# KochPJ/AutoPoseEstimation

Measured on AMD Instinct MI355X. Metric: RGB-D frames/sec (seg+DenseFusion+2-refine), 640x480 N=1000, higher is better.
Workload: dtype bf16x3

## Files before the change

autoposeestimation_amd/_lib.py:

```python
import ctypes
import os

import torch

_HERE = os.path.dirname(os.path.abspath(__file__))
LIB_PATH = os.environ.get("APE_HIP_LIB", os.path.join(_HERE, "libape_hip.so"))

_c = ctypes
_P, _I, _F, _L, _D = _c.c_void_p, _c.c_int, _c.c_float, _c.c_int64, _c.c_double

SIGNATURES = {
    "ape_abi_version": [],
    "ape_last_error": [],
    "ape_knn_f32": [_P, _P, _P, _I, _I, _I, _I, _I, _P],
    "ape_conv2d_nhwc_f32": [_P, _P, _P, _P, _P, _P, _P],
    "ape_packed_weights_bf16_elems": [_I, _I],
    "ape_pack_weights_bf16": [_P, _P, _I, _I, _P],
    "ape_conv2d_nhwc_bf16": [_P, _P, _P, _P, _P, _P, _I, _P],
    "ape_conv_gemm_supported": [_P],
    "ape_conv_gemm_bf16": [_P, _P, _P, _P, _P, _P, _I, _I, _P],
    "ape_pack_weights_s32k": [_P, _P, _I, _I, _P],
    "ape_convert_s32": [_P, _P, _c.c_long, _I, _I, _P],
    "ape_conv_gemm_s32_supported": [_P],
    "ape_conv_gemm_s32_debug": [_I],
    "ape_conv3x3_halo_s32_debug": [_I],
    "ape_conv_gemm_s32": [_P, _P, _P, _P, _I, _P, _I, _P, _P],
    "ape_conv_gemm_s32_per_image": [_P, _P, _c.c_long, _P, _P, _I, _P, _P],
    "ape_psp_fold_operands": [_P, _P, _P, _P, _P, _P, _P, _I, _I, _I, _I, _I, _I, _P],
    "ape_conv_gemm_bf16_fmt": [_P, _P, _P, _P, _P, _I, _P, _I, _I, _P],
    "ape_conv_gemm_splitk_workspace_bytes": [_P],
    "ape_conv_gemm_bf16_splitk": [_P, _P, _P, _P, _P, _P, _I, _P, _c.c_size_t, _P],
    "ape_conv_gemm_bf16_multi": [_I, _P, _P, _P, _P, _P, _I, _P],
    "ape_adaptive_avgpool_multi_nhwc_ld": [_P, _I, _P, _P, _I, _I, _I, _I, _I, _I, _P, _c.c_size_t, _P],
    "ape_upconv3x3_gather_ex": [_P, _P, _P, _I, _I, _I, _I, _I, _I, _F, _I, _P],
    "ape_upconv3x3_gather_strip_rows": [_I],
    "ape_upconv3x3_fused_supported": [_I, _I, _I, _I],
    "ape_upconv3x3_fused_debug": [_I],
    "ape_upconv3x3_fused_stamps": [_P],
    "ape_upconv3x3_fused_s32": [_P, _P, _P, _P, _I, _I, _I, _I, _I, _I, _F, _I, _P],
    "ape_upconv3x3_fused_seghead_s32": [_P, _P, _P, _I, _I, _I, _I, _I, _F, _I, _P, _P, _I, _P, _P, _I, _P],
    "ape_conv3x3_halo_s32_supported": [_P],
    "ape_conv3x3_halo_s32": [_P, _P, _P, _P, _I, _P, _I, _P, _P],
    "ape_conv3x3_halo_mx_supported": [_P],
    "ape_conv3x3_halo_mx": [_P, _P, _P, _P, _I, _P, _I, _P, _P],
    "ape_conv3x3_halo_mx_debug": [_I],
    "ape_s32_to_f16m6": [_P, _P, _c.c_long, _I, _P],
    "ape_stem_conv_pool_bf16": [_P, _P, _P, _P, _I, _I, _I, _I, _P],
    "ape_stem_conv_pool_u8": [_P, _I, _P, _P, _P, _P, _I, _I, _I, _I, _I, _I, _I, _P],
    "ape_conv3x3_halo_supported": [_P],
    "ape_conv3x3_halo_bf16": [_P, _P, _P, _P, _P, _P, _I, _P],
    "ape_maxpool3x3s2_nhwc_f32": [_P, _P, _I, _I, _I, _I, _P],
    "ape_adaptive_avgpool_nhwc_f32": [_P, _P, _I, _I, _I, _I, _I, _P],
    "ape_adaptive_avgpool_multi_workspace_bytes": [_I, _I],
    "ape_bilinear_nhwc_f32": [_P, _P, _I, _I, _I, _I, _I, _I, _I, _I, _I, _I, _I, _P],
    "ape_psp_prior_sum_f32": [_P, _P, _P, _P, _P, _I, _I, _I, _I, _P],
    "ape_upconv3x3_gather_f32": [_P, _P, _P, _I, _I, _I, _I, _I, _F, _P],
    "ape_gather_rows_f32": [_P, _P, _P, _I, _I, _I, _I, _P],
    "ape_ups_patch_gather_f32": [_P, _P, _P, _I, _I, _I, _I, _I, _P],
    "ape_log_softmax_rows_f32": [_P, _P, _c.c_long, _I, _P],
    "ape_mean_rows_f32": [_P, _P, _I, _I, _I, _P],
    "ape_pad3to4_f32": [_P, _P, _c.c_long, _P],
    "ape_head_select_f32": [_P, _I, _I, _I, _I, _P, _P, _P, _P, _P, _P, _P, _P, _I, _I, _I, _P],
    "ape_pose_select_f32": [_P, _P, _P, _P, _P, _I, _I, _P],
    "ape_head_conf_argmax_f32": [_P, _I, _I, _P, _P, _P, _P, _P, _P, _I, _P, _I, _I, _I, _P],
    "ape_pose_from_row_f32": [_P, _I, _I, _I, _P, _P, _P, _P, _P, _P, _P, _P, _P, _I, _I, _I, _P],
    "ape_pose_compose_f64": [_P, _P, _I, _P, _I, _I, _P],
    "ape_pose_recentre_f32": [_P, _P, _P, _I, _I, _P],
    "ape_adds_dis_f32": [_P, _P, _P, _P, _P, _I, _I, _I, _P, _P, _P, _P],
    "ape_adds_dis_batched_f32": [_P, _P, _P, _P, _I, _I, _I, _P, _P, _P],
    "ape_adds_select_f32": [_P, _P, _P, _P, _P, _P, _I, _F, _P, _P, _P],
    "ape_recentre_qt_f32": [_P, _P, _P, _I, _P],
    "ape_pose_errors_chunk": [],
    "ape_pose_errors_queries": [],
    "ape_pose_errors_lanes": [_c.c_long, _I],
    "ape_pose_errors_workspace_bytes": [_c.c_long, _I],
    "ape_pose_errors_f64": [_P, _P, _I, _c.c_long, _P, _P, _P, _P, _c.c_long, _I, _I, _P, _P, _c.c_size_t, _P],
    "ape_seg_argmax_f32": [_P, _I, _I, _P, _P, _c.c_long, _I, _P],
    "ape_seg_head_f32": [_P, _P, _P, _I, _P, _P, _c.c_long, _I, _P],
    "ape_seg_components_workspace_bytes": [_I, _I, _I, _I],
    "ape_conv3x3_halo_seghead_bf16": [_P, _P, _P, _P, _I, _P, _P, _I, _P, _P, _I, _P],
    "ape_unet_conv3x3_supported": [_I, _I, _I, _I],
    "ape_unet_conv3x3_bf16": [_P, _I, _I, _P, _I, _I, _P, _P, _P, _I, _I, _I, _I, _I, _I, _I, _I, _P],
    "ape_unet_conv3x3_seghead_bf16": [_P, _I, _I, _P, _I, _I, _P, _P, _I, _P, _P, _I, _I, _I, _I, _I, _I, _P],
    "ape_nearest_upsample_nhwc_f32": [_P, _P, _I, _I, _I, _I, _I, _I, _I, _P],
    "ape_seg_components_scored": [_P, _P, _P, _P, _I, _I, _I, _I, _I, _I, _P, _c.c_size_t, _P],
    "ape_bgsub_features_f32": [_P, _P, _P, _P, _P, _P, _P, _P, _P, _I, _I, _I, _P],
    "ape_conv2d_wgrad_workspace_bytes": [_P],
    "ape_conv2d_wgrad_nhwc_f32": [_P, _P, _P, _P, _P, _c.c_size_t, _P],
# ... 132 lines not shown
                                          "KH", "KW", "stride", "pad", "dil", "act")] + \
               [("alpha", _c.c_float), ("bias_bstride", _c.c_int32), ("ldr", _c.c_int32), ("roff", _c.c_int32), ("ups", _c.c_int32)]


class AugRotation(_c.Structure):
    _fields_ = [("a", _c.c_double * 6), ("fa", _c.c_int32 * 6), ("mode", _c.c_int32), ("reserved", _c.c_int32)]


class AugJitter(_c.Structure):
    _fields_ = [("n_ops", _c.c_int32), ("code", _c.c_int32 * 4), ("factor", _c.c_float * 4), ("shift", _c.c_int32 * 4)]


class BgsubTrainJob(_c.Structure):
    _fields_ = [("f_rgb", _c.c_void_p), ("b_rgb", _c.c_void_p), ("f_depth", _c.c_void_p), ("b_depth", _c.c_void_p), ("label", _c.c_void_p),
                ("rot", AugRotation), ("jit", AugJitter * 2), ("hflip", _c.c_int32), ("vflip", _c.c_int32)]


class SegTrainJob(_c.Structure):
    _fields_ = [("rgb", _c.c_void_p), ("label", _c.c_void_p), ("rot", AugRotation), ("jit", AugJitter), ("crop_x", _c.c_int32),
                ("crop_y", _c.c_int32), ("crop_side", _c.c_int32), ("class_id", _c.c_int32)]


class PoseTrainJob(_c.Structure):
    _fields_ = [("rgb", _c.c_void_p), ("depth", _c.c_void_p), ("label", _c.c_void_p), ("rot", AugRotation), ("add_t", _c.c_double * 3),
                ("out_off", _c.c_longlong), ("jit", AugJitter), ("rmin", _c.c_int32), ("rmax", _c.c_int32), ("cmin", _c.c_int32),
                ("cmax", _c.c_int32), ("ppx", _c.c_float), ("ppy", _c.c_float), ("fx", _c.c_float), ("fy", _c.c_float),
                ("depth_scale", _c.c_float), ("to_meter", _c.c_int32), ("add_noise", _c.c_int32)]


ACT_NONE, ACT_RELU, ACT_PRELU, ACT_SIGMOID = 0, 1, 2, 3
_RESTYPES = {"ape_last_error": _c.c_char_p, "ape_adaptive_avgpool_multi_workspace_bytes": _c.c_size_t, "ape_seg_components_workspace_bytes": _c.c_size_t,
             "ape_packed_weights_bf16_elems": _c.c_long, "ape_pc_batch_workspace_bytes": _c.c_size_t,
             "ape_conv2d_wgrad_workspace_bytes": _c.c_size_t, "ape_conv_gemm_splitk_workspace_bytes": _c.c_size_t,
             "ape_fpfh_workspace_bytes": _c.c_size_t, "ape_feature_nn1_workspace_bytes": _c.c_size_t, "ape_ransac_workspace_bytes": _c.c_size_t,
             "ape_fpfh_batch_workspace_bytes": _c.c_size_t, "ape_feature_nn1_batch_workspace_bytes": _c.c_size_t,
             "ape_ransac_batch_workspace_bytes": _c.c_size_t,
             "ape_bn_workspace_bytes": _c.c_size_t, "ape_jaccard_workspace_bytes": _c.c_size_t,
             "ape_bgsub_train_workspace_bytes": _c.c_size_t, "ape_seg_train_workspace_bytes": _c.c_size_t,
             "ape_seg_train_extents_offset": _c.c_size_t, "ape_seg_train_tables_offset": _c.c_size_t,
             "ape_pose_train_extents_offset": _c.c_size_t, "ape_pose_train_rows_offset": _c.c_size_t,
             "ape_pose_train_tables_offset": _c.c_size_t, "ape_pose_train_sel_offset": _c.c_size_t,
             "ape_pose_train_workspace_bytes": _c.c_size_t, "ape_pose_train_image_offset": _c.c_size_t,
             "ape_pose_train_sample_bytes": _c.c_size_t,
             "ape_linemod_box_workspace_bytes": _c.c_size_t, "ape_linemod_rows_offset": _c.c_size_t,
             "ape_linemod_tables_offset": _c.c_size_t, "ape_linemod_sel_offset": _c.c_size_t, "ape_linemod_workspace_bytes": _c.c_size_t,
             "ape_ycb_rows_offset": _c.c_size_t, "ape_ycb_tables_offset": _c.c_size_t, "ape_ycb_sel_offset": _c.c_size_t,
             "ape_ycb_noise_offset": _c.c_size_t, "ape_pose_errors_workspace_bytes": _c.c_size_t,
             "ape_cross_entropy_workspace_bytes": _c.c_size_t, "ape_segnet_samples_frames_offset": _c.c_size_t,
             "ape_rgbd_cca_workspace_bytes": _c.c_size_t}

_lib = None


ABI_VERSION = 18


class ApeError(RuntimeError):
    code = None


def lib():
    global _lib
    if _lib is None:
        if not os.path.exists(LIB_PATH):
            raise ImportError(
                "%s not found: build it with `python -c 'import __graft_entry__ as g; g.build()'` "
                "or `make -C autoposeestimation_amd/csrc` (hipcc, gfx950). There is no CPU fallback." % LIB_PATH)
        h = ctypes.CDLL(LIB_PATH)
        h.ape_abi_version.restype = _c.c_int
        if h.ape_abi_version() != ABI_VERSION:
            raise ImportError("%s is ABI %d, this package expects ABI %d: a stale library -- rebuild it with "
                              "`python -c 'import __graft_entry__ as g; g.build()'`" % (LIB_PATH, h.ape_abi_version(), ABI_VERSION))
        for name, argtypes in SIGNATURES.items():
            fn = getattr(h, name)
            fn.argtypes = argtypes
            fn.restype = _RESTYPES.get(name, _c.c_int)
        _lib = h
    return _lib


_raw_stream = getattr(torch._C, "_cuda_getCurrentRawStream", None)
_get_device = getattr(torch._C, "_cuda_getDevice", None) or torch.cuda.current_device


def stream_ptr():
    if _raw_stream is not None:
        return _c.c_void_p(_raw_stream(_get_device()))
    return _c.c_void_p(torch.cuda.current_stream().cuda_stream)


def dptr(t, dtype=None):
    if t is None:
        return _c.c_void_p(0)
    if not t.is_cuda:
        raise ApeError("tensor is on %s; the HIP path needs device memory (no CPU fallback)" % t.device)
    if not t.is_contiguous():
        raise ApeError("tensor must be contiguous")
    if dtype is not None and t.dtype != dtype:
        raise ApeError("expected %s, got %s" % (dtype, t.dtype))
    return _c.c_void_p(t.data_ptr())


def _failed(what, rc):
    msg = lib().ape_last_error()
    err = ApeError("%s failed: code %d (%s)" % (what, rc, msg.decode() if msg else ""))
    err.code = rc
    return err
# ... 28 lines not shown
```

autoposeestimation_amd/csrc/ops.hip:

```cpp
#include <map>
#include <mutex>
#include "s32.h"

namespace {

using ape::src_index;
constexpr int kThreads = 256;
constexpr int kGridCap = 8192;

__global__ void maxpool3x3s2_kernel(const float4* __restrict__ x, float4* __restrict__ y, int B, int H, int W, int C4,
                                    int Ho, int Wo)
{
    const long total = (long)B * Ho * Wo * C4;
    for (long i = blockIdx.x * (long)blockDim.x + threadIdx.x; i < total; i += (long)gridDim.x * blockDim.x) {
        const int c = i % C4;
        long t = i / C4;
        const int ox = t % Wo; t /= Wo;
        const int oy = t % Ho;
        const int b = t / Ho;
        float4 m = make_float4(-__builtin_inff(), -__builtin_inff(), -__builtin_inff(), -__builtin_inff());
#pragma unroll
        for (int ky = 0; ky < 3; ++ky) {
            const int iy = oy * 2 - 1 + ky;
            if ((unsigned)iy >= (unsigned)H) continue;
// ... 368 lines not shown
                if (FMA) {
                    acc.x = fmaf(ly1[ky], v1[u][ky].x, fmaf(ly0[ky], v0[u][ky].x, acc.x));
                    acc.y = fmaf(ly1[ky], v1[u][ky].y, fmaf(ly0[ky], v0[u][ky].y, acc.y));
                    acc.z = fmaf(ly1[ky], v1[u][ky].z, fmaf(ly0[ky], v0[u][ky].z, acc.z));
                    acc.w = fmaf(ly1[ky], v1[u][ky].w, fmaf(ly0[ky], v0[u][ky].w, acc.w));
                    continue;
                }
                acc.x += ly0[ky] * v0[u][ky].x + ly1[ky] * v1[u][ky].x;
                acc.y += ly0[ky] * v0[u][ky].y + ly1[ky] * v1[u][ky].y;
                acc.z += ly0[ky] * v0[u][ky].z + ly1[ky] * v1[u][ky].z;
                acc.w += ly0[ky] * v0[u][ky].w + ly1[ky] * v1[u][ky].w;
            }
            if (sidx[u] >= 0) S[sidx[u]] = acc;
        }
    }
    __syncthreads();
    for (int item = threadIdx.x; item < 16 * C4; item += 256) {
        const int c = item % C4;
        const int X = X0 + item / C4;
        if (X >= Wo) continue;
        float4 acc = make_float4(0.f, 0.f, 0.f, 0.f);
#pragma unroll
        for (int kx = 0; kx < 3; ++kx) {
            const int qx = X + kx - 1;
            if ((unsigned)qx >= (unsigned)Wo) continue;
            const float fx = sw * (float)qx;
            const int ix0 = (int)fx, ix1 = ix0 + (ix0 < w - 1 ? 1 : 0);
            const float lx1 = fx - (float)ix0, lx0 = 1.f - lx1;
            const float4 s0 = S[(kx * kUpCols + ix0 - ix_lo) * C4 + c], s1 = S[(kx * kUpCols + ix1 - ix_lo) * C4 + c];
            if (FMA) {
                acc.x = fmaf(lx1, s1.x, fmaf(lx0, s0.x, acc.x));
                acc.y = fmaf(lx1, s1.y, fmaf(lx0, s0.y, acc.y));
                acc.z = fmaf(lx1, s1.z, fmaf(lx0, s0.z, acc.z));
                acc.w = fmaf(lx1, s1.w, fmaf(lx0, s0.w, acc.w));
                continue;
            }
            acc.x += lx0 * s0.x + lx1 * s1.x;
            acc.y += lx0 * s0.y + lx1 * s1.y;
            acc.z += lx0 * s0.z + lx1 * s1.z;
            acc.w += lx0 * s0.w + lx1 * s1.w;
        }
        if (bias) { acc.x += bias[c * 4]; acc.y += bias[c * 4 + 1]; acc.z += bias[c * 4 + 2]; acc.w += bias[c * 4 + 3]; }
        if (act == APE_ACT_RELU) { acc.x = fmaxf(acc.x, 0.f); acc.y = fmaxf(acc.y, 0.f); acc.z = fmaxf(acc.z, 0.f); acc.w = fmaxf(acc.w, 0.f); }
        else if (act == APE_ACT_PRELU) {
            acc.x = acc.x > 0.f ? acc.x : alpha * acc.x; acc.y = acc.y > 0.f ? acc.y : alpha * acc.y;
            acc.z = acc.z > 0.f ? acc.z : alpha * acc.z; acc.w = acc.w > 0.f ? acc.w : alpha * acc.w;
        }
        if (S32OUT) ape::s32_store4(out, (long)(b * Ho + Y) * Wo + X, C4, c, acc);
        else out[((long)(b * Ho + Y) * Wo + X) * C4 + c] = acc;
    }
}

typedef float ups_f32x2 __attribute__((ext_vector_type(2)));
template <bool S32OUT, bool FMA>
__global__ __launch_bounds__(256) void upconv_gather_strip_kernel(const float4* __restrict__ z, const float* __restrict__ bias,
                                                                  float4* __restrict__ out, int B, int h, int w, int C4, float sh, float sw,
                                                                  int act, float alpha, int rows)
{
    const int Ho = 2 * h, Wo = 2 * w;
    const int xt_n = (Wo + 15) / 16, ns = (Ho + rows - 1) / rows, nslab = C4 / 16;
    const int nwg = gridDim.x;
    const int orig = blockIdx.x;
    const int xcd = orig % 8, q = nwg / 8, r = nwg % 8;
    int logical = (xcd < r ? xcd * (q + 1) : r * (q + 1) + (xcd - r) * q) + orig / 8;
    const int slab = logical % nslab; logical /= nslab;
    const int xt = logical % xt_n; logical /= xt_n;
    const int strip = logical % ns;
    const int b = logical / ns;
    const int Ys = strip * rows, Ye = Ys + rows < Ho ? Ys + rows : Ho;
    __shared__ float4 S[2][3 * kUpCols * 16];
    const int X0 = xt * 16;
    const int qx_lo = X0 - 1 < 0 ? 0 : X0 - 1, qx_hi = X0 + 16 > Wo - 1 ? Wo - 1 : X0 + 16;
    const int ix_lo = (int)(sw * (float)qx_lo);
    int ix_hi = (int)(sw * (float)qx_hi);
    ix_hi = ix_hi + (ix_hi < w - 1 ? 1 : 0);
    const int ni = ix_hi - ix_lo + 1;
    const int c4 = threadIdx.x & 15, hi4 = threadIdx.x >> 4;
    const int c = slab * 16 + c4;
    constexpr int NIT = 3;
    bool p1[NIT];
    int it_s[NIT];
    const long rs = (long)w * 9 * C4;
    const float4* zi[NIT];
#pragma unroll
    for (int r = 0; r < NIT; ++r) {
        const int item = hi4 + 16 * r;
        p1[r] = item < 3 * ni;
        const int col = p1[r] ? item / 3 : 0, kx = p1[r] ? item - 3 * col : 0;
        it_s[r] = (kx * kUpCols + col) * 16 + c4;
        zi[r] = z + (long)b * h * rs + (long)(ix_lo + col) * 9 * C4 + kx * C4 + c;
    }
    const bool third = __builtin_amdgcn_readfirstlane((int)(threadIdx.x >> 6)) * 4 + 32 < 3 * ni;
    float4 v0[3][NIT], v1[3][NIT];
    int hy0[3];
    const int X = X0 + hi4;
    const bool p2 = X < Wo;
    int so0[3], so1[3];
    float lx0[3], lx1[3];
    bool xok[3];
#pragma unroll
    for (int kx = 0; kx < 3; ++kx) {
        const int qx = X + kx - 1;
        xok[kx] = p2 && (unsigned)qx < (unsigned)Wo;
        const float fx = sw * (float)(xok[kx] ? qx : 0);
        const int ix0 = (int)fx, ix1 = ix0 + (ix0 < w - 1 ? 1 : 0);
        lx1[kx] = fx - (float)ix0;
        lx0[kx] = 1.f - lx1[kx];
        so0[kx] = xok[kx] ? (kx * kUpCols + ix0 - ix_lo) * 16 + c4 : c4;
        so1[kx] = xok[kx] ? (kx * kUpCols + ix1 - ix_lo) * 16 + c4 : c4;
    }
    float4 bv = make_float4(0.f, 0.f, 0.f, 0.f);
    if (bias) bv = make_float4(bias[c * 4], bias[c * 4 + 1], bias[c * 4 + 2], bias[c * 4 + 3]);

#define APE_UPS_ROWS(YY, ky, iy0, iy1)                                                                                                     \
    const int qy_##ky = (YY) + (ky) - 1;                                                                                                   \
    const int iy0 = __builtin_amdgcn_readfirstlane((int)(sh * (float)((unsigned)qy_##ky < (unsigned)Ho ? qy_##ky : 0)));                   \
    const int iy1 = iy0 + (iy0 < h - 1 ? 1 : 0);
#define APE_UPS_ADVANCE(YY, ky)                                                                                                            \
    {                                                                                                                                      \
        APE_UPS_ROWS(YY, ky, iy0, iy1)                                                                                                     \
        const bool keep = iy0 == hy0[ky];                                                                                                  \
        const long o1 = (long)iy1 * rs + (ky) * 3 * C4;                                                                                    \
        _Pragma("unroll") for (int r = 0; r < NIT; ++r) {                                                                                  \
// ... 22 lines not shown
            ly1[ky] = fy - (float)(int)fy;                                                                                                 \
            ly0[ky] = 1.f - ly1[ky];                                                                                                       \
        }                                                                                                                                  \
        _Pragma("unroll") for (int kx = 0; kx < NIT; ++kx) {                                     \
            if (kx == 2 && !third) break;                                                                                                  \
            float4 acc = make_float4(0.f, 0.f, 0.f, 0.f);                                                                                  \
            _Pragma("unroll") for (int ky = 0; ky < 3; ++ky) {                                                                             \
                if (!yok[ky]) continue;                                                                                                    \
                const float4 a0 = v0[ky][kx], a1 = v1[ky][kx];                                                                             \
                if (FMA) {                                                                                                                 \
                    acc.x = fmaf(ly1[ky], a1.x, fmaf(ly0[ky], a0.x, acc.x));                                                               \
                    acc.y = fmaf(ly1[ky], a1.y, fmaf(ly0[ky], a0.y, acc.y));                                                               \
                    acc.z = fmaf(ly1[ky], a1.z, fmaf(ly0[ky], a0.z, acc.z));                                                               \
                    acc.w = fmaf(ly1[ky], a1.w, fmaf(ly0[ky], a0.w, acc.w));                                                               \
                    continue;                                                                                                              \
                }                                                                                                                          \
                          \
                const ups_f32x2 w0 = {ly0[ky], ly0[ky]}, w1 = {ly1[ky], ly1[ky]};                                                          \
                const ups_f32x2 tl = w0 * ups_f32x2{a0.x, a0.y} + w1 * ups_f32x2{a1.x, a1.y};                                              \
                const ups_f32x2 th = w0 * ups_f32x2{a0.z, a0.w} + w1 * ups_f32x2{a1.z, a1.w};                                              \
                const ups_f32x2 sl = ups_f32x2{acc.x, acc.y} + tl, sh2 = ups_f32x2{acc.z, acc.w} + th;                                     \
                acc = make_float4(sl.x, sl.y, sh2.x, sh2.y);                                                                               \
            }                                                                                                                              \
            if (p1[kx]) (Sb)[it_s[kx]] = acc;                                                                                              \
        }                                                                                                                                  \
    }
#define APE_UPS_PHASE2(YY, Sb)                                                                                                             \
    if (p2) {                                                                                                                              \
        float4 acc = make_float4(0.f, 0.f, 0.f, 0.f);                                                                                      \
        _Pragma("unroll") for (int kx = 0; kx < 3; ++kx) {                                                                                 \
            if (!xok[kx]) continue;                                                                                                        \
            const float4 s0 = (Sb)[so0[kx]], s1 = (Sb)[so1[kx]];                                                                           \
            if (FMA) {                                                                                                                     \
                acc.x = fmaf(lx1[kx], s1.x, fmaf(lx0[kx], s0.x, acc.x));                                                                   \
                acc.y = fmaf(lx1[kx], s1.y, fmaf(lx0[kx], s0.y, acc.y));                                                                   \
                acc.z = fmaf(lx1[kx], s1.z, fmaf(lx0[kx], s0.z, acc.z));                                                                   \
                acc.w = fmaf(lx1[kx], s1.w, fmaf(lx0[kx], s0.w, acc.w));                                                                   \
                continue;                                                                                                                  \
            }                                                                                                                              \
            {                                                                                                                              \
                const ups_f32x2 w0 = {lx0[kx], lx0[kx]}, w1 = {lx1[kx], lx1[kx]};                                                          \
                const ups_f32x2 tl = w0 * ups_f32x2{s0.x, s0.y} + w1 * ups_f32x2{s1.x, s1.y};                                              \
                const ups_f32x2 th = w0 * ups_f32x2{s0.z, s0.w} + w1 * ups_f32x2{s1.z, s1.w};                                              \
                const ups_f32x2 sl = ups_f32x2{acc.x, acc.y} + tl, sh2 = ups_f32x2{acc.z, acc.w} + th;                                     \
                acc = make_float4(sl.x, sl.y, sh2.x, sh2.y);                                                                               \
            }                                                                                                                              \
        }                                                                                                                                  \
        if (bias) { acc.x += bv.x; acc.y += bv.y; acc.z += bv.z; acc.w += bv.w; }                                                          \
        if (act == APE_ACT_RELU) { acc.x = fmaxf(acc.x, 0.f); acc.y = fmaxf(acc.y, 0.f); acc.z = fmaxf(acc.z, 0.f); acc.w = fmaxf(acc.w, 0.f); } \
        else if (act == APE_ACT_PRELU) {                                                                                                   \
            acc.x = acc.x > 0.f ? acc.x : alpha * acc.x; acc.y = acc.y > 0.f ? acc.y : alpha * acc.y;                                      \
            acc.z = acc.z > 0.f ? acc.z : alpha * acc.z; acc.w = acc.w > 0.f ? acc.w : alpha * acc.w;                                      \
        }                                                                                                                                  \
        if (S32OUT) ape::s32_store4_pair(out, (long)(b * Ho + (YY)) * Wo + X, C4, c, acc);     \
        else out[((long)(b * Ho + (YY)) * Wo + X) * C4 + c] = acc;                                                                         \
    }

    APE_UPS_INIT(Ys, 0) APE_UPS_INIT(Ys, 1) APE_UPS_INIT(Ys, 2)
    for (int Y = Ys; Y < Ye; Y += 2) {
        APE_UPS_PHASE1(Y, S[0])
        APE_UPS_ADVANCE(Y + 1, 1)
        __syncthreads();
        APE_UPS_PHASE2(Y, S[0])
        APE_UPS_PHASE1(Y + 1, S[1])
        APE_UPS_ADVANCE(Y + 2, 0)
        APE_UPS_ADVANCE(Y + 2, 2)
        __syncthreads();
        APE_UPS_PHASE2(Y + 1, S[1])
    }
#undef APE_UPS_ROWS
#undef APE_UPS_ADVANCE
#undef APE_UPS_INIT
#undef APE_UPS_PHASE1
#undef APE_UPS_PHASE2
}

__global__ void psp_prior_sum_kernel(const float4* __restrict__ z1, const float4* __restrict__ z2, const float4* __restrict__ z3,
                                     const float4* __restrict__ z6, float4* __restrict__ out, int B, int h, int w, int C4)
{
    const long total = (long)B * w * C4;
    for (long i = blockIdx.x * (long)blockDim.x + threadIdx.x; i < total; i += (long)gridDim.x * blockDim.x) {
        const int c = i % C4;
        const long t = i / C4;
        const int ox = t % w;
        const int b = t / w;
        float4 tx[12];
        const float4* zs[4] = {z1, z2, z3, z6};
        const int ss[4] = {1, 2, 3, 6};
        const int base[4] = {0, 1, 3, 6};
#pragma unroll
        for (int k = 0; k < 4; ++k) {
            const int S = ss[k];
            const float fx = src_index(ox, (float)S / (float)w, false);
            const int ix0 = (int)fx;
            const int ix1 = ix0 + (ix0 < S - 1 ? 1 : 0);
            const float lx1 = fx - (float)ix0, lx0 = 1.f - lx1;
            const float4* z = zs[k] + (long)b * S * S * C4 + c;
#pragma unroll
            for (int iy = 0; iy < S; ++iy) {
                const float4 v0 = z[(iy * S + ix0) * C4], v1 = z[(iy * S + ix1) * C4];
                tx[base[k] + iy] = make_float4(lx0 * v0.x + lx1 * v1.x, lx0 * v0.y + lx1 * v1.y, lx0 * v0.z + lx1 * v1.z,
                                               lx0 * v0.w + lx1 * v1.w);
            }
        }
        float4* o = out + ((long)b * h * w + ox) * C4 + c;
        for (int oy = 0; oy < h; ++oy) {
            float4 acc = make_float4(0.f, 0.f, 0.f, 0.f);
#pragma unroll
            for (int k = 0; k < 4; ++k) {
                const int S = ss[k];
                const float fy = src_index(oy, (float)S / (float)h, false);
                const int iy0 = (int)fy;
                const int iy1 = iy0 + (iy0 < S - 1 ? 1 : 0);
                const float ly1 = fy - (float)iy0, ly0 = 1.f - ly1;
                float4 t0 = tx[base[k]], t1 = tx[base[k]];
#pragma unroll
                for (int r = 0; r < S; ++r) {
                    if (r == iy0) t0 = tx[base[k] + r];
                    if (r == iy1) t1 = tx[base[k] + r];
                }
                acc.x += ly0 * t0.x + ly1 * t1.x;
                acc.y += ly0 * t0.y + ly1 * t1.y;
                acc.z += ly0 * t0.z + ly1 * t1.z;
                acc.w += ly0 * t0.w + ly1 * t1.w;
            }
// ... 151 lines not shown
    if (B == 0) return APE_OK;
    if (C % 4 == 0 && n >= 64)
        hipLaunchKernelGGL(mean_rows_wide_kernel, dim3(ape::ceil_div(C / 4, 64), B), dim3(1024), 0, (hipStream_t)stream,
                           (const float4*)x, (float4*)y, n, C / 4);
    else
        hipLaunchKernelGGL(mean_rows_kernel, dim3(ape::ceil_div(C, 64), B), dim3(256), 0, (hipStream_t)stream, x, y, n, C);
    return ape::check_launch("ape_mean_rows_f32");
}

extern "C" int ape_pad3to4_f32(const float* x, float* y, long rows, void* stream)
{
    if (!x || !y || rows < 0) return APE_EINVAL;
    if (rows == 0) return APE_OK;
    hipLaunchKernelGGL(pad3to4_kernel, dim3(ape::grid_for(rows, kThreads, kGridCap)), dim3(kThreads), 0, (hipStream_t)stream, x, (float4*)y, rows);
    return ape::check_launch("ape_pad3to4_f32");
}

extern "C" int ape_head_select_f32(const float* h, int ldh, int off_r, int off_t, int off_c, const float* wr, const float* br,
                                   const float* wt, const float* bt, const float* wc, const float* bc, const int64_t* obj,
                                   float* out, int B, int n, int K, void* stream)
{
    if (!h || !wr || !br || !wt || !bt || (wc && !bc) || !obj || !out || B < 0 || n < 0 || K < 1 || K > 1024) return APE_EINVAL;
    if (B == 0 || n == 0) return APE_OK;
    dim3 grid(ape::ceil_div((long)n * 8, kThreads), B);
    hipLaunchKernelGGL(head_select_kernel, grid, dim3(kThreads), 8 * K * sizeof(float), (hipStream_t)stream, h, ldh, off_r,
                       off_t, off_c, wr, br, wt, bt, wc, bc, obj, out, n, K);
    return ape::check_launch("ape_head_select_f32");
}

extern "C" int ape_upconv3x3_gather_f32(const float* z, const float* bias, float* out, int B, int h, int w, int C, int act, float alpha,
                                        void* stream)
{
    return ape_upconv3x3_gather_ex(z, bias, out, APE_FMT_F32, B, h, w, C, act, alpha, 0, stream);
}

static bool strip_schedule_ok(int h, float sh)
{
    static std::mutex mu;
    static std::map<int, bool> seen;
    std::lock_guard<std::mutex> lock(mu);
    auto it = seen.find(h);
    if (it != seen.end()) return it->second;
    bool ok = true;
    int prev = (int)(sh * 0.f);
    for (int q = 1; q < 2 * h && ok; ++q) {
        const int cur = (int)(sh * (float)q);
        ok = (q & 1) ? (cur == prev || cur == prev + 1) : cur == prev;
        prev = cur;
    }
    seen[h] = ok;
    return ok;
}

static int g_upg_strip_rows = 30;
extern "C" int ape_upconv3x3_gather_strip_rows(int rows)
{
    const int old = g_upg_strip_rows;
    if (rows >= 0) g_upg_strip_rows = rows;
    return old;
}

extern "C" int ape_upconv3x3_gather_ex(const float* z, const float* bias, void* out, int out_fmt, int B, int h, int w, int C, int act,
                                       float alpha, int fma, void* stream)
{
    if ((out_fmt != APE_FMT_F32 && out_fmt != APE_FMT_S32) || (out_fmt == APE_FMT_S32 && C % 32) || (fma != 0 && fma != 1)) return APE_EINVAL;
    if (!z || !out || B < 0 || h < 1 || w < 1 || C < 4 || C % 4 || act < APE_ACT_NONE || act > APE_ACT_PRELU) return APE_EINVAL;
    const long total = (long)B * 4 * h * w * (C / 4);
    if (total == 0) return APE_OK;
    const float sh = 2 * h > 1 ? (float)(h - 1) / (float)(2 * h - 1) : 0.f;
    const float sw = 2 * w > 1 ? (float)(w - 1) / (float)(2 * w - 1) : 0.f;
    if (C % 64 == 0 && g_upg_strip_rows > 0 && strip_schedule_ok(h, sh)) {
        const int rows = (g_upg_strip_rows + 1) & ~1;
        const long gs = (long)B * ((2 * h + rows - 1) / rows) * ((2 * w + 15) / 16) * (C / 64);
        if (gs >= (1L << 31)) return APE_EINVAL;
#define APE_UPS_LAUNCH(S32O, FM)                                                                                                           \
    hipLaunchKernelGGL((upconv_gather_strip_kernel<S32O, FM>), dim3((unsigned)gs), dim3(256), 0, (hipStream_t)stream, (const float4*)z,    \
                       bias, (float4*)out, B, h, w, C / 4, sh, sw, act, alpha, rows)
        if (out_fmt == APE_FMT_S32) { if (fma) APE_UPS_LAUNCH(true, true); else APE_UPS_LAUNCH(true, false); }
        else { if (fma) APE_UPS_LAUNCH(false, true); else APE_UPS_LAUNCH(false, false); }
#undef APE_UPS_LAUNCH
        return ape::check_launch("ape_upconv3x3_gather_f32");
    }
    const long g = (long)B * 2 * h * ((2 * w + 15) / 16);
    if (g >= (1L << 31)) return APE_EINVAL;
    const size_t lds = (size_t)3 * kUpCols * (C / 4) * sizeof(float4);
    if (lds > 64 * 1024) return APE_EINVAL;
#define APE_UPG_LAUNCH(S32O, FM)                                                                                                          \
    hipLaunchKernelGGL((upconv_gather_kernel<S32O, FM>), dim3((unsigned)g), dim3(256), lds, (hipStream_t)stream, (const float4*)z, bias, \
                       (float4*)out, B, h, w, C / 4, sh, sw, act, alpha)
    if (out_fmt == APE_FMT_S32) { if (fma) APE_UPG_LAUNCH(true, true); else APE_UPG_LAUNCH(true, false); }
    else { if (fma) APE_UPG_LAUNCH(false, true); else APE_UPG_LAUNCH(false, false); }
#undef APE_UPG_LAUNCH
    return ape::check_launch("ape_upconv3x3_gather_f32");
}

extern "C" int ape_psp_prior_sum_f32(const float* z1, const float* z2, const float* z3, const float* z6, float* out, int B, int h,
                                     int w, int C, void* stream)
{
    if (!z1 || !z2 || !z3 || !z6 || !out || B < 0 || h < 1 || w < 1 || C < 4 || C % 4) return APE_EINVAL;
    const long total = (long)B * w * (C / 4);
    if (total == 0) return APE_OK;
    hipLaunchKernelGGL(psp_prior_sum_kernel, dim3(ape::grid_for(total, kThreads, kGridCap)), dim3(kThreads), 0, (hipStream_t)stream, (const float4*)z1,
                       (const float4*)z2, (const float4*)z3, (const float4*)z6, (float4*)out, B, h, w, C / 4);
    return ape::check_launch("ape_psp_prior_sum_f32");
}
```

autoposeestimation_amd/csrc/runtime.hip:

```cpp
#include "common.h"
#include <string.h>

namespace ape {
static thread_local char g_err[256] = "";
void set_last_error(const char* what)
{
    strncpy(g_err, what ? what : "", sizeof(g_err) - 1);
    g_err[sizeof(g_err) - 1] = 0;
}
}

extern "C" int ape_abi_version(void) { return 18; }
extern "C" const char* ape_last_error(void) { return ape::g_err; }
```

autoposeestimation_amd/engine.py:

```python
import contextlib
import contextvars
import ctypes
import os

import torch

from . import _lib
from ._lib import ACT_NONE, ACT_PRELU, ACT_RELU, ACT_SIGMOID, ConvParams


def _st():
    return _lib.stream_ptr()


class LaunchProfile:

    def __init__(self, only=None):
        self.records = []
        self.only = only

    def wants(self, label):
        return self.only is None or label in self.only

    def begin(self, label):
# ... 609 lines not shown
    b, c = zs[0].shape[0], zs[0].shape[3]
    out = torch.empty(b, h, w, c, dtype=torch.float32, device=zs[0].device)
    _lib.call.ape_psp_prior_sum_f32(*[_lib.dptr(z, torch.float32) for z in zs], _lib.dptr(out), b, h, w, c, _st())
    return out


USE_PSP_FOLD = os.environ.get("APE_USE_PSP_FOLD", "1") != "0"
PSP_FOLD_K = 64


def psp_bottleneck_folded(conv, x576, zs, out_fmt=FMT_S32):
    xt = x576.t
    b, h, w, ld = xt.shape
    if conv.nsplit != 3 or (conv.kh, conv.kw, conv.stride, conv.pad) != (1, 1, 1, 0) or ld != conv.cin + PSP_FOLD_K or [tuple(z.shape) for z in zs] != [(b, s, s, conv.cout) for s in (1, 2, 3, 6)]:
        raise ValueError("psp_bottleneck_folded: a split-bf16 1x1 layer, an S32 map of Cin + 64 channels and the four prior maps [B,s,s,Cout]")
    groups = conv.cin // 32 + 2
    wimg = torch.empty(b, conv.cout, groups * 64, dtype=torch.bfloat16, device=xt.device)
    _lib.call.ape_psp_fold_operands(_lib.dptr(conv.s32k()), *[_lib.dptr(z, torch.float32) for z in zs], _lib.dptr(wimg),
                                    _lib.dptr(xt, torch.float32), b, h, w, ld, conv.cin, conv.cout, _st())
    out = torch.empty(b, h, w, conv.cout, dtype=torch.float32, device=xt.device)
    p = conv_params(conv, b, h, w, ld, conv.cout)
    p.Cin = ld
    label = gemm_s32_label(conv.cout)
    e0 = _prof_begin(label)
    _lib.call.ape_conv_gemm_s32_per_image(_lib.dptr(xt, torch.float32), _lib.dptr(wimg), conv.cout * groups * 128, _lib.dptr(conv.bias),
                                          _lib.dptr(out), out_fmt, ctypes.byref(p), _st())
    if e0 is not None:
        _prof_end(e0, label, "%dx%dx%d %d+%d->%d k1 s1 d1 psp-fold" % (b, h, w, conv.cin, PSP_FOLD_K, conv.cout), 2.0 * b * h * w * conv.cout * ld,
                  4.0 * (b * h * w * ld + b * conv.cout * ld + b * h * w * conv.cout))
    return S32(out) if out_fmt == FMT_S32 else out


USE_UPFUSE = os.environ.get("APE_USE_UPFUSE", "1") != "0"


class UpConv:

    def __init__(self, weight, bias, alpha, device="cuda", precision="f32", fma=False, splitk=False):
        cout, cin, kh, kw = weight.shape
        assert (kh, kw) == (3, 3)
        w9 = weight.detach().permute(2, 3, 0, 1).reshape(9 * cout, cin)
        self.mix = Conv(w9, None, device=device, precision=precision, splitk=splitk)
        self.bias = bias.detach().to(device=device, dtype=torch.float32).contiguous()
        self.alpha, self.cout, self.cin, self.fma = float(alpha), cout, cin, bool(fma)

    def fusable(self, x):
        return bool(USE_UPFUSE and isinstance(x, S32) and self.mix.nsplit == 3 and x.shape[3] == self.cin
                    and _lib.lib().ape_upconv3x3_fused_supported(x.shape[1], x.shape[2], self.cin, self.cout))

    def _gather(self, z, out_fmt):
        b, h, w, _ = z.shape
        out = torch.empty(b, 2 * h, 2 * w, self.cout, dtype=torch.float32, device=z.device)
        strip = self.cout % 64 == 0 and _lib.lib().ape_upconv3x3_gather_strip_rows(-1) > 0
        glabel = "upconv_gather_%skernel<%s,%s>" % ("strip_" if strip else "", "true" if out_fmt == FMT_S32 else "false", "true" if self.fma else "false")
        e0 = _prof_begin(glabel)
        _lib.call.ape_upconv3x3_gather_ex(_lib.dptr(z, torch.float32), _lib.dptr(self.bias), _lib.dptr(out), out_fmt, b, h, w,
                                          self.cout, ACT_PRELU, self.alpha, int(self.fma), _st())
        if e0 is not None:
            _prof_end(e0, glabel, "%dx%dx%d C%d" % (b, 2 * h, 2 * w, self.cout), 0.0, 4.0 * (b * h * w * 9 * self.cout + b * 4 * h * w * self.cout))
        return S32(out) if out_fmt == FMT_S32 else out

    def __call__(self, x, out_fmt=FMT_F32, fused=None):
        if fused is None:
            fused = self.fusable(x)
        if not fused:
            return self._gather(self.mix(x), out_fmt)
        if not self.fusable(x):
            raise ValueError("no fused PSPUpsample kernel for this layer / input (needs split-bf16 operands, an S32 input, 64 -> 64 channels)")
        b, h, w, _ = x.shape
        out = torch.empty(b, 2 * h, 2 * w, self.cout, dtype=torch.float32, device=x.device)
        label = "upconv_fused_kernel<%d,false,%s>" % (self.cin // 32, "true" if self.fma else "false")
        e0 = _prof_begin(label)
        _lib.call.ape_upconv3x3_fused_s32(_lib.dptr(x.t, torch.float32), _lib.dptr(self.mix.s32k()), _lib.dptr(self.bias), _lib.dptr(out),
                                          out_fmt, b, h, w, self.cin, ACT_PRELU, self.alpha, int(self.fma), _st())
        if e0 is not None:
            _prof_end(e0, label, "%dx%dx%d %d->%d up (executed flop; direct form x4)" % (b, 2 * h, 2 * w, self.cin, self.cout), *self._fused_cost(b, h, w, 4.0 * self.cout))
        return S32(out) if out_fmt == FMT_S32 else out

    def _fused_cost(self, b, h, w, out_bytes_per_pixel):
        return (2.0 * b * h * w * 9 * self.cout * self.cin,
                4.0 * (b * h * w * self.cin + 9 * self.cout * self.cin) + out_bytes_per_pixel * b * 4 * h * w)

    def seg_head(self, x, head_w, head_b, double_softmax=True, fused=None):
        if fused is None:
            fused = self.fusable(x) and head_w.shape[0] <= 16 and self.cout == 64
        if not fused:
            return seg_head(self(x, fused=False), head_w, head_b, double_softmax)
        b, h, w, _ = x.shape
        c = head_w.shape[0]
        label = torch.empty(b, 2 * h, 2 * w, dtype=torch.uint8, device=x.device)
        score = torch.empty(b, 2 * h, 2 * w, dtype=torch.float32, device=x.device)
        klabel = "upconv_fused_kernel<%d,true,%s>" % (self.cin // 32, "true" if self.fma else "false")
        e0 = _prof_begin(klabel)
        _lib.call.ape_upconv3x3_fused_seghead_s32(_lib.dptr(x.t, torch.float32), _lib.dptr(self.mix.s32k()), _lib.dptr(self.bias), b, h, w,
                                                  self.cin, ACT_PRELU, self.alpha, int(self.fma), _lib.dptr(head_w, torch.float32),
                                                  _lib.dptr(head_b), c, _lib.dptr(label), _lib.dptr(score), int(bool(double_softmax)), _st())
        if e0 is not None:
            _prof_end(e0, klabel, "%dx%dx%d %d->%d up +head (executed flop; direct form x4)" % (b, 2 * h, 2 * w, self.cin, self.cout), *self._fused_cost(b, h, w, 5.0))
        return label, score


def gather_rows(x, index):
    b, r, c = x.shape
    n = index.shape[1]
    y = torch.empty(b, n, c, dtype=torch.float32, device=x.device)
    _lib.call.ape_gather_rows_f32(_lib.dptr(x, torch.float32), _lib.dptr(index, torch.int64), _lib.dptr(y), b, r, n, c, _st())
    return y
# ... 458 lines not shown
```

include/ape_hip.h:

```cpp
#ifndef APE_HIP_H
#define APE_HIP_H

#include <stddef.h>
#include <stdint.h>

#ifdef __cplusplus
extern "C" {
#define APE_STATIC_ASSERT static_assert
#else
#define APE_STATIC_ASSERT _Static_assert
#endif

#define APE_OK 0
#define APE_EINVAL (-1)
#define APE_ELAUNCH (-2)
#define APE_EWORKSPACE (-3)

int ape_abi_version(void);
const char* ape_last_error(void);

int ape_knn_f32(const float* ref, const float* query, int64_t* idx,
                int batch, int dim, int ref_nb, int query_nb, int k, void* stream);

enum { APE_ACT_NONE = 0, APE_ACT_RELU = 1, APE_ACT_PRELU = 2, APE_ACT_SIGMOID = 3 };
typedef struct ape_conv_params {
    int32_t B, H, W, Cin, ldx, xoff;
    int32_t Ho, Wo, Cout, ldy, yoff;
    int32_t KH, KW, stride, pad, dil;
    int32_t act;
    float alpha;
    int32_t bias_bstride;
    int32_t ldr, roff;
    int32_t ups;
} ape_conv_params;
int ape_conv2d_nhwc_f32(const float* x, const float* w, const float* bias, const float* residual, float* y,
                        const ape_conv_params* params_host, void* stream);

long ape_packed_weights_bf16_elems(int cout, int K);
int ape_pack_weights_bf16(const float* w, void* out, int cout, int K, void* stream);
int ape_conv2d_nhwc_bf16(const float* x, const void* w_packed, const float* bias, const float* residual, float* y,
                         const ape_conv_params* params_host, int nsplit, void* stream);
int ape_conv_gemm_supported(const ape_conv_params* params_host);
int ape_conv_gemm_bf16(const float* x, const void* w_packed, const float* bias, const float* residual, float* y,
                       const ape_conv_params* params_host, int nsplit, int variant, void* stream);
enum { APE_FMT_F32 = 0, APE_FMT_S32 = 1 };
int ape_pack_weights_s32k(const float* w, void* out, int cout, int K, void* stream);
int ape_convert_s32(const void* x, void* y, long rows, int C, int to_s32, void* stream);
int ape_conv_gemm_s32_supported(const ape_conv_params* params_host);
int ape_conv3x3_halo_s32_debug(int bits);
int ape_conv_gemm_s32_debug(int bits);
int ape_conv_gemm_s32(const void* x_s32, const void* w_s32k, const float* bias, const void* residual, int res_fmt, void* y,
                      int out_fmt, const ape_conv_params* params_host, void* stream);
int ape_conv_gemm_s32_per_image(const void* x_s32, const void* w_s32k, long w_image_stride_bytes, const float* bias, void* y, int out_fmt,
                                const ape_conv_params* params_host, void* stream);
int ape_psp_fold_operands(const void* wf_s32k, const float* z1, const float* z2, const float* z3, const float* z6, void* w_out, void* x_s32,
                          int B, int h, int w, int ld, int Cin, int Cout, void* stream);
int ape_conv_gemm_bf16_fmt(const float* x, const void* w_packed, const float* bias, const float* residual, void* y, int out_fmt,
                           const ape_conv_params* params_host, int nsplit, int variant, void* stream);
int ape_conv_gemm_bf16_multi(int n, const float* const* x, const void* const* w_packed, const float* const* bias, float* const* y,
                             const ape_conv_params* params_host, int nsplit, void* stream);
size_t ape_conv_gemm_splitk_workspace_bytes(const ape_conv_params* params);
int ape_conv_gemm_bf16_splitk(const float* x, const void* w_packed, const float* bias, const float* residual, float* y,
                              const ape_conv_params* params, int nsplit, void* workspace, size_t workspace_bytes, void* stream);
int ape_adaptive_avgpool_multi_nhwc_ld(const void* x, int in_fmt, float* const* ys_host, const int* sizes_host, int nsizes, int B, int H, int W,
                                       int C, int ldx, void* workspace, size_t workspace_bytes, void* stream);
int ape_upconv3x3_gather_ex(const float* z, const float* bias, void* out, int out_fmt, int B, int h, int w, int C, int act, float alpha,
                            int fma, void* stream);
int ape_upconv3x3_gather_strip_rows(int rows);
int ape_upconv3x3_fused_supported(int h, int w, int Cin, int Cout);
int ape_upconv3x3_fused_stamps(void* device_buffer);
int ape_upconv3x3_fused_debug(int bits);
int ape_upconv3x3_fused_s32(const void* x_s32, const void* w9_s32k, const float* bias, void* out, int out_fmt, int B, int h, int w, int Cin,
                            int act, float alpha, int fma, void* stream);
int ape_upconv3x3_fused_seghead_s32(const void* x_s32, const void* w9_s32k, const float* bias, int B, int h, int w, int Cin, int act, float alpha,
                                    int fma, const float* head_w, const float* head_b, int C, uint8_t* label, float* score, int double_softmax,
                                    void* stream);
int ape_conv3x3_halo_s32_supported(const ape_conv_params* params_host);
int ape_conv3x3_halo_s32(const void* x_s32, const void* w_s32k, const float* bias, const void* residual, int res_fmt, void* y,
                         int out_fmt, const ape_conv_params* params_host, void* stream);
int ape_conv3x3_halo_mx_supported(const ape_conv_params* params_host);
int ape_conv3x3_halo_mx(const void* x_f16m6, const void* w_f16m6, const float* bias, const void* residual, int res_fmt, void* y,
                        int out_fmt, const ape_conv_params* params_host, void* stream);
int ape_conv3x3_halo_mx_debug(int bits);
int ape_s32_to_f16m6(const void* x_s32, void* y_f16m6, long pixels, int C, void* stream);
int ape_stem_conv_pool_bf16(const float* x, const float* w, const float* bias, float* y, int B, int H, int W, int nsplit,
                            void* stream);
int ape_stem_conv_pool_u8(const uint8_t* rgb, int n_frames, const int* rects, const float* w, const float* bias, float* y, int n, int Hf, int Wf,
                          int Hc, int Wc, int div255, int nsplit, void* stream);
int ape_conv3x3_halo_supported(const ape_conv_params* params_host);
int ape_conv3x3_halo_bf16(const float* x, const void* w_packed, const float* bias, const float* residual, float* y,
                          const ape_conv_params* params_host, int nsplit, void* stream);

int ape_maxpool3x3s2_nhwc_f32(const float* x, float* y, int B, int H, int W, int C, void* stream);
int ape_adaptive_avgpool_nhwc_f32(const float* x, float* y, int B, int H, int W, int C, int S, void* stream);
size_t ape_adaptive_avgpool_multi_workspace_bytes(int B, int C);
int ape_bilinear_nhwc_f32(const float* x, float* y, int B, int H, int W, int C, int ldx, int Ho, int Wo, int ldy,
                          int yoff, int align_corners, int accumulate, void* stream);
int ape_psp_prior_sum_f32(const float* z1, const float* z2, const float* z3, const float* z6, float* out, int B, int h,
                          int w, int C, void* stream);
int ape_upconv3x3_gather_f32(const float* z, const float* bias, float* out, int B, int h, int w, int C, int act, float alpha,
                             void* stream);
int ape_gather_rows_f32(const float* x, const int64_t* index, float* y, int B, int rows_in, int n, int C, void* stream);
int ape_ups_patch_gather_f32(const float* x, const int64_t* index, float* out, int B, int h, int w, int C, int n, void* stream);
int ape_log_softmax_rows_f32(const float* x, float* y, long rows, int C, void* stream);
int ape_mean_rows_f32(const float* x, float* y, int B, int n, int C, void* stream);
int ape_pad3to4_f32(const float* x, float* y, long rows, void* stream);
int ape_head_select_f32(const float* h, int ldh, int off_r, int off_t, int off_c, const float* wr, const float* br,
                        const float* wt, const float* bt, const float* wc, const float* bc, const int64_t* obj,
                        float* out, int B, int n, int K, void* stream);

int ape_pose_select_f32(const float* heads, const float* points4, double* pose, int* which, float* new_points4,
                        int B, int n, void* stream);
int ape_head_conf_argmax_f32(const float* h3c, int ldh, int off_c, const float* wc, const float* bc, const int64_t* obj,
                             int* which_out, float* conf_out, const float* pf, int ld_pf, float* pf_row_out, int B, int n, int K,
                             void* stream);
int ape_pose_from_row_f32(const float* h3rt_row, int ldh, int off_r, int off_t, const float* wr, const float* br, const float* wt,
                          const float* bt, const int64_t* obj, const int* which, const float* points4, double* pose,
                          float* new_points4, int B, int n, int K, void* stream);
int ape_pose_compose_f64(double* pose, const float* ref_r, int ldr, const float* ref_t, int ldt, int B, void* stream);
int ape_pose_recentre_f32(const float* points4, const double* pose, float* new_points4, int B, int n, void* stream);

// ... 378 lines not shown
```

Measured before the change: 2101.

## Add register-prefetching upconv gather kernel that loads next input rows ahead

```diff
diff --git a/autoposeestimation_amd/_lib.py b/autoposeestimation_amd/_lib.py
--- a/autoposeestimation_amd/_lib.py
+++ b/autoposeestimation_amd/_lib.py
@@ -34,6 +34,7 @@
     "ape_adaptive_avgpool_multi_nhwc_ld": [_P, _I, _P, _P, _I, _I, _I, _I, _I, _I, _P, _c.c_size_t, _P],
     "ape_upconv3x3_gather_ex": [_P, _P, _P, _I, _I, _I, _I, _I, _I, _F, _I, _P],
     "ape_upconv3x3_gather_strip_rows": [_I],
+    "ape_upconv3x3_gather_debug": [_I],
     "ape_upconv3x3_fused_supported": [_I, _I, _I, _I],
     "ape_upconv3x3_fused_debug": [_I],
     "ape_upconv3x3_fused_stamps": [_P],
@@ -272,7 +273,7 @@
 _lib = None
 
 
-ABI_VERSION = 18
+ABI_VERSION = 19
 
 
 class ApeError(RuntimeError):
diff --git a/autoposeestimation_amd/csrc/ops.hip b/autoposeestimation_amd/csrc/ops.hip
--- a/autoposeestimation_amd/csrc/ops.hip
+++ b/autoposeestimation_amd/csrc/ops.hip
@@ -444,6 +444,17 @@
 }
 
 typedef float ups_f32x2 __attribute__((ext_vector_type(2)));
+#if defined(APE_ABLATIONS)
+#define APE_UPS_ABL(bit) (dbg & (bit))
+#else
+#define APE_UPS_ABL(bit) 0
+#endif
+__device__ __forceinline__ void ups_keep(const float4& v)
+{
+#if defined(__HIP_DEVICE_COMPILE__)
+    asm volatile("" ::"v"(v.x), "v"(v.y), "v"(v.z), "v"(v.w));
+#endif
+}
 template <bool S32OUT, bool FMA>
 __global__ __launch_bounds__(256) void upconv_gather_strip_kernel(const float4* __restrict__ z, const float* __restrict__ bias,
                                                                   float4* __restrict__ out, int B, int h, int w, int C4, float sh, float sw,
@@ -461,6 +472,7 @@
     const int b = logical / ns;
     const int Ys = strip * rows, Ye = Ys + rows < Ho ? Ys + rows : Ho;
     __shared__ float4 S[2][3 * kUpCols * 16];
+    [[maybe_unused]] constexpr int dbg = 0;
     const int X0 = xt * 16;
     const int qx_lo = X0 - 1 < 0 ? 0 : X0 - 1, qx_hi = X0 + 16 > Wo - 1 ? Wo - 1 : X0 + 16;
     const int ix_lo = (int)(sw * (float)qx_lo);
@@ -589,7 +601,8 @@
             acc.x = acc.x > 0.f ? acc.x : alpha * acc.x; acc.y = acc.y > 0.f ? acc.y : alpha * acc.y;                                      \
             acc.z = acc.z > 0.f ? acc.z : alpha * acc.z; acc.w = acc.w > 0.f ? acc.w : alpha * acc.w;                                      \
         }                                                                                                                                  \
-        if (S32OUT) ape::s32_store4_pair(out, (long)(b * Ho + (YY)) * Wo + X, C4, c, acc);     \
+        if (APE_UPS_ABL(8)) ups_keep(acc);                                                                    \
+        else if (S32OUT) ape::s32_store4_pair(out, (long)(b * Ho + (YY)) * Wo + X, C4, c, acc);     \
         else out[((long)(b * Ho + (YY)) * Wo + X) * C4 + c] = acc;                                                                         \
     }
 
@@ -605,9 +618,135 @@
         __syncthreads();
         APE_UPS_PHASE2(Y + 1, S[1])
     }
-#undef APE_UPS_ROWS
 #undef APE_UPS_ADVANCE
 #undef APE_UPS_INIT
+}
+
+constexpr int kUpKxCols = 10;
+__device__ __forceinline__ void ups_move(float4& dst, const float4& src)
+{
+#if defined(__HIP_DEVICE_COMPILE__)
+    asm volatile("v_mov_b32 %0, %4\n\tv_mov_b32 %1, %5\n\tv_mov_b32 %2, %6\n\tv_mov_b32 %3, %7"
+                 : "=&v"(dst.x), "=&v"(dst.y), "=&v"(dst.z), "=&v"(dst.w) : "v"(src.x), "v"(src.y), "v"(src.z), "v"(src.w) : "memory");
+#else
+    dst = src;
+#endif
+}
+__device__ __forceinline__ void ups_arrived(float4& v)
+{
+#if defined(__HIP_DEVICE_COMPILE__)
+    asm volatile("" : "+v"(v.x), "+v"(v.y), "+v"(v.z), "+v"(v.w));
+#endif
+}
+template <bool S32OUT, bool FMA>
+__global__ __launch_bounds__(256) void upconv_gather_ahead_kernel(const float4* __restrict__ z, const float* __restrict__ bias,
+                                                                  float4* __restrict__ out, int B, int h, int w, int C4, float sh, float sw,
+                                                                  int act, float alpha, int rows, int dbg)
+{
+    const int Ho = 2 * h, Wo = 2 * w;
+    const int xt_n = (Wo + 15) / 16, ns = (Ho + rows - 1) / rows, nslab = C4 / 16;
+    const int nwg = gridDim.x;
+    const int orig = blockIdx.x;
+    const int xcd = orig % 8, q = nwg / 8, r = nwg % 8;
+    int logical = (xcd < r ? xcd * (q + 1) : r * (q + 1) + (xcd - r) * q) + orig / 8;
+    const int slab = logical % nslab; logical /= nslab;
+    const int xt = logical % xt_n; logical /= xt_n;
+    const int strip = logical % ns;
+    const int b = logical / ns;
+    const int Ys = strip * rows, Ye = Ys + rows < Ho ? Ys + rows : Ho;
+    __shared__ float4 S[2][3 * kUpCols * 16];
+    const int X0 = xt * 16, X1 = X0 + 15 < Wo - 1 ? X0 + 15 : Wo - 1;
+    const int ix_lo = (int)(sw * (float)(X0 - 1 < 0 ? 0 : X0 - 1));
+    const int c4 = threadIdx.x & 15, hi4 = threadIdx.x >> 4;
+    const int c = slab * 16 + c4;
+    constexpr int NIT = 2;
+    constexpr bool third = false;
+    bool p1[NIT];
+    int it_s[NIT];
+    const long rs = (long)w * 9 * C4;
+    const float4* zi[NIT];
+#pragma unroll
+    for (int r = 0; r < NIT; ++r) {
+        const int item = hi4 + 16 * r;
+        const int kx = item / kUpKxCols < 2 ? item / kUpKxCols : 2, ci = item - kx * kUpKxCols;
+        const int q_lo = X0 + kx - 1 < 0 ? 0 : X0 + kx - 1, q_hi = X1 + kx - 1 > Wo - 1 ? Wo - 1 : X1 + kx - 1;
+        const int k_lo = (int)(sw * (float)q_lo);
+        int k_hi = (int)(sw * (float)q_hi);
+        k_hi = k_hi + (k_hi < w - 1 ? 1 : 0);
+        p1[r] = ci < kUpKxCols && k_lo + ci <= k_hi;
+        const int col = p1[r] ? k_lo + ci : k_lo;
+        it_s[r] = (kx * kUpCols + col - ix_lo) * 16 + c4;
+        zi[r] = z + (long)b * h * rs + (long)col * 9 * C4 + kx * C4 + c;
+    }
+    float4 v0[3][NIT], v1[3][NIT], nx[3][NIT];
+    int hy0[3];
+    const int X = X0 + hi4;
+    const bool p2 = X < Wo;
+    int so0[3], so1[3];
+    float lx0[3], lx1[3];
+    bool xok[3];
+#pragma unroll
+    for (int kx = 0; kx < 3; ++kx) {
+        const int qx = X + kx - 1;
+        xok[kx] = p2 && (unsigned)qx < (unsigned)Wo;
+        const float fx = sw * (float)(xok[kx] ? qx : 0);
+        const int ix0 = (int)fx, ix1 = ix0 + (ix0 < w - 1 ? 1 : 0);
+        lx1[kx] = fx - (float)ix0;
+        lx0[kx] = 1.f - lx1[kx];
+        so0[kx] = xok[kx] ? (kx * kUpCols + ix0 - ix_lo) * 16 + c4 : c4;
+        so1[kx] = xok[kx] ? (kx * kUpCols + ix1 - ix_lo) * 16 + c4 : c4;
+    }
+    float4 bv = make_float4(0.f, 0.f, 0.f, 0.f);
+    if (bias) bv = make_float4(bias[c * 4], bias[c * 4 + 1], bias[c * 4 + 2], bias[c * 4 + 3]);
+
+#define APE_UPA_REQUEST(YN, ky)                                                                                                            \
+    {                                                                                                                                      \
+        APE_UPS_ROWS(YN, ky, jy0, jy1)                                                                                                     \
+        const long on = (long)jy1 * rs + (ky) * 3 * C4;                                                                                    \
+        _Pragma("unroll") for (int r = 0; r < NIT; ++r) nx[ky][r] = zi[r][on];                                                             \
+    }
+#define APE_UPA_ADVANCE(YY, ky)                                                                                                            \
+    {                                                                                                                                      \
+        APE_UPS_ROWS(YY, ky, iy0, iy1)                                                                                                     \
+        (void)iy1;                                                                                        \
+        const bool keep = iy0 == hy0[ky];                                                                                                  \
+        _Pragma("unroll") for (int r = 0; r < NIT; ++r) {                                                                                  \
+            v0[ky][r].x = keep ? v0[ky][r].x : v1[ky][r].x; v0[ky][r].y = keep ? v0[ky][r].y : v1[ky][r].y;                                \
+            v0[ky][r].z = keep ? v0[ky][r].z : v1[ky][r].z; v0[ky][r].w = keep ? v0[ky][r].w : v1[ky][r].w;                                \
+            ups_move(v1[ky][r], nx[ky][r]);                                                                                                \
+        }                                                                                                                                  \
+        hy0[ky] = iy0;                                                                                                                     \
+        if (!APE_UPS_ABL(1)) APE_UPA_REQUEST((YY) + 2, ky)                                                                                 \
+    }
+#define APE_UPA_INIT(YY, ky)                                                                                                               \
+    {                                                                                                                                      \
+        APE_UPS_ROWS(YY, ky, iy0, iy1)                                                                                                     \
+        const long o0 = (long)iy0 * rs + (ky) * 3 * C4, o1 = (long)iy1 * rs + (ky) * 3 * C4;                                               \
+        _Pragma("unroll") for (int r = 0; r < NIT; ++r) { v0[ky][r] = zi[r][o0]; v1[ky][r] = zi[r][o1]; }                                  \
+        hy0[ky] = iy0;                                                                                                                     \
+    }
+
+    APE_UPA_INIT(Ys, 0) APE_UPA_INIT(Ys, 1) APE_UPA_INIT(Ys, 2)
+    APE_UPA_REQUEST(Ys + 1, 1) APE_UPA_REQUEST(Ys + 2, 0) APE_UPA_REQUEST(Ys + 2, 2)
+#pragma unroll
+    for (int ky = 0; ky < 3; ++ky)
+#pragma unroll
+        for (int r = 0; r < NIT; ++r) { ups_arrived(v0[ky][r]); ups_arrived(v1[ky][r]); ups_arrived(nx[ky][r]); }
+    for (int Y = Ys; Y < Ye; Y += 2) {
+        if (!APE_UPS_ABL(2)) APE_UPS_PHASE1(Y, S[0])
+        APE_UPA_ADVANCE(Y + 1, 1)
+        __syncthreads();
+        if (!APE_UPS_ABL(4)) APE_UPS_PHASE2(Y, S[0])
+        if (!APE_UPS_ABL(2)) APE_UPS_PHASE1(Y + 1, S[1])
+        APE_UPA_ADVANCE(Y + 2, 0)
+        APE_UPA_ADVANCE(Y + 2, 2)
+        __syncthreads();
+        if (!APE_UPS_ABL(4)) APE_UPS_PHASE2(Y + 1, S[1])
+    }
+#undef APE_UPA_REQUEST
+#undef APE_UPA_ADVANCE
+#undef APE_UPA_INIT
+#undef APE_UPS_ROWS
 #undef APE_UPS_PHASE1
 #undef APE_UPS_PHASE2
 }
@@ -865,6 +1004,38 @@
     return ok;
 }
 
+static bool strip_cols_ok(int w, float sw)
+{
+    static std::mutex mu;
+    static std::map<int, bool> seen;
+    std::lock_guard<std::mutex> lock(mu);
+    auto it = seen.find(w);
+    if (it != seen.end()) return it->second;
+    const int Wo = 2 * w;
+    bool ok = true;
+    for (int X0 = 0; X0 < Wo && ok; X0 += 16) {
+        const int X1 = X0 + 15 < Wo - 1 ? X0 + 15 : Wo - 1;
+        const int ix_lo = (int)(sw * (float)(X0 - 1 < 0 ? 0 : X0 - 1));
+        for (int kx = 0; kx < 3 && ok; ++kx) {
+            const int q_lo = X0 + kx - 1 < 0 ? 0 : X0 + kx - 1, q_hi = X1 + kx - 1 > Wo - 1 ? Wo - 1 : X1 + kx - 1;
+            const int k_lo = (int)(sw * (float)q_lo);
+            int k_hi = (int)(sw * (float)q_hi);
+            k_hi = k_hi + (k_hi < w - 1 ? 1 : 0);
+            ok = q_lo <= q_hi && k_lo >= ix_lo && k_hi - k_lo + 1 <= kUpKxCols && k_hi - ix_lo < kUpCols;
+        }
+    }
+    seen[w] = ok;
+    return ok;
+}
+
+static int g_upg_debug = 0;
+extern "C" int ape_upconv3x3_gather_debug(int bits)
+{
+    const int old = g_upg_debug;
+    if (bits >= 0) g_upg_debug = bits;
+    return old;
+}
+
 static int g_upg_strip_rows = 30;
 extern "C" int ape_upconv3x3_gather_strip_rows(int rows)
 {
@@ -886,6 +1057,15 @@
         const int rows = (g_upg_strip_rows + 1) & ~1;
         const long gs = (long)B * ((2 * h + rows - 1) / rows) * ((2 * w + 15) / 16) * (C / 64);
         if (gs >= (1L << 31)) return APE_EINVAL;
+        if (!(g_upg_debug & 1) && strip_cols_ok(w, sw)) {
+#define APE_UPA_LAUNCH(S32O, FM)                                                                                                           \
+    hipLaunchKernelGGL((upconv_gather_ahead_kernel<S32O, FM>), dim3((unsigned)gs), dim3(256), 0, (hipStream_t)stream, (const float4*)z,    \
+                       bias, (float4*)out, B, h, w, C / 4, sh, sw, act, alpha, rows, g_upg_debug >> 4)
+            if (out_fmt == APE_FMT_S32) { if (fma) APE_UPA_LAUNCH(true, true); else APE_UPA_LAUNCH(true, false); }
+            else { if (fma) APE_UPA_LAUNCH(false, true); else APE_UPA_LAUNCH(false, false); }
+#undef APE_UPA_LAUNCH
+            return ape::check_launch("ape_upconv3x3_gather_f32");
+        }
 #define APE_UPS_LAUNCH(S32O, FM)                                                                                                           \
     hipLaunchKernelGGL((upconv_gather_strip_kernel<S32O, FM>), dim3((unsigned)gs), dim3(256), 0, (hipStream_t)stream, (const float4*)z,    \
                        bias, (float4*)out, B, h, w, C / 4, sh, sw, act, alpha, rows)
diff --git a/autoposeestimation_amd/csrc/runtime.hip b/autoposeestimation_amd/csrc/runtime.hip
--- a/autoposeestimation_amd/csrc/runtime.hip
+++ b/autoposeestimation_amd/csrc/runtime.hip
@@ -10,5 +10,5 @@
 }
 }
 
-extern "C" int ape_abi_version(void) { return 18; }
+extern "C" int ape_abi_version(void) { return 19; }
 extern "C" const char* ape_last_error(void) { return ape::g_err; }
diff --git a/autoposeestimation_amd/engine.py b/autoposeestimation_amd/engine.py
--- a/autoposeestimation_amd/engine.py
+++ b/autoposeestimation_amd/engine.py
@@ -685,7 +685,8 @@
         b, h, w, _ = z.shape
         out = torch.empty(b, 2 * h, 2 * w, self.cout, dtype=torch.float32, device=z.device)
         strip = self.cout % 64 == 0 and _lib.lib().ape_upconv3x3_gather_strip_rows(-1) > 0
-        glabel = "upconv_gather_%skernel<%s,%s>" % ("strip_" if strip else "", "true" if out_fmt == FMT_S32 else "false", "true" if self.fma else "false")
+        form = ("ahead_" if not _lib.lib().ape_upconv3x3_gather_debug(-1) & 1 else "strip_") if strip else ""
+        glabel = "upconv_gather_%skernel<%s,%s>" % (form, "true" if out_fmt == FMT_S32 else "false", "true" if self.fma else "false")
         e0 = _prof_begin(glabel)
         _lib.call.ape_upconv3x3_gather_ex(_lib.dptr(z, torch.float32), _lib.dptr(self.bias), _lib.dptr(out), out_fmt, b, h, w,
                                           self.cout, ACT_PRELU, self.alpha, int(self.fma), _st())
diff --git a/include/ape_hip.h b/include/ape_hip.h
--- a/include/ape_hip.h
+++ b/include/ape_hip.h
@@ -31,8 +31,7 @@
     float alpha;
     int32_t bias_bstride;
     int32_t ldr, roff;
-    int32_t ups;
-} ape_conv_params;
+    int32_t ups;            } ape_conv_params;
 int ape_conv2d_nhwc_f32(const float* x, const float* w, const float* bias, const float* residual, float* y,
                         const ape_conv_params* params_host, void* stream);
 
@@ -67,6 +66,7 @@
 int ape_upconv3x3_gather_ex(const float* z, const float* bias, void* out, int out_fmt, int B, int h, int w, int C, int act, float alpha,
                             int fma, void* stream);
 int ape_upconv3x3_gather_strip_rows(int rows);
+int ape_upconv3x3_gather_debug(int bits);
 int ape_upconv3x3_fused_supported(int h, int w, int Cin, int Cout);
 int ape_upconv3x3_fused_stamps(void* device_buffer);
 int ape_upconv3x3_fused_debug(int bits);
```

New measurement: 2101. No clear change (-0.0%).
